# mFinn27/Template-Matching-and-Regression-MapReduce

Measured on AMD Instinct MI355X. Metric: images/sec (whole node) match+regress+NMS; % HBM/MFMA roofline at 1/2/4/8 GPU, higher is better.
Workload: dtype fp32; 1 GPU; config B: 64x SAM feats 256x64x64 (->128x128), 3 exemplars, templates 3x3-15x15, fp32, cls 0.1, IoU 0.5; config=B, images_per_gpu=64, exemplars=3, parallelism=dp1, decoder=split, decoder_precision=fp32

## Files before the change

template-matching-and-regression-mapreduce_amd/csrc/conv_split.hip:

```cpp
#include <algorithm>
#include <type_traits>

#include "tmr_common.h"

namespace {

typedef _Float16 h8 __attribute__((ext_vector_type(8)));
typedef __bf16 b8 __attribute__((ext_vector_type(8)));
typedef float f32x4 __attribute__((ext_vector_type(4)));
typedef __bf16 b4 __attribute__((ext_vector_type(4)));
typedef __attribute__((address_space(3))) void *lds_ptr_t;


constexpr int BM = 128;
constexpr int TH = 16;
constexpr int TW = 32;
constexpr int LDS_KB = 160;
constexpr int PXG = 8, NG = 4;
constexpr int NWAVES = 8;
constexpr int NTHREADS = NWAVES * 64;
constexpr int WNS = (NWAVES == 8 || TH == 8) ? 2 : 1;
static_assert(TH == 4 * NWAVES / WNS, "a wave owns 4 output rows");
constexpr int NIN = 8 / WNS;
constexpr int ACCW = NIN * 8 * 64 * 4;
// ... 473 lines not shown
    if (EPI == 0 && (a.flags & TMR_SPLIT_TILED_OUT)) {
        f32x4 *o = reinterpret_cast<f32x4 *>(
                       a.out + ((((size_t)u * a.NT + nt) * a.MT + mt) * NWAVES + wave) * ACCW) +
                   lane;
#pragma unroll
        for (int in = 0; in < NIN; ++in)
#pragma unroll
            for (int jp = 0; jp < 8; ++jp) {
                __builtin_nontemporal_store(acc[in][jp] * inv, o + (in * 8 + jp) * 64);
            }
        return;
    }
    float *red = reinterpret_cast<float *>(lds);
    float *sb = red + 4 * 8 * NHEAD * 16;
    float *shw = sb + BM;
    if (tid < BM) {
        const int n = nt * BM + tid;
        sb[tid] = n < a.N ? a.bias[n] : 0.0f;
    }
    if (EPI == 1)
        for (int e = tid; e < BM * NHEAD; e += NTHREADS) shw[e] = a.headw[(size_t)nt * BM * NHEAD + e];
    __syncthreads();
    if constexpr (EPI == 0) {
        float invp[8];
#pragma unroll
        for (int jp = 0; jp < 8; ++jp) {
            invp[jp] = inv;
            const int y = ty0 + wpix * 4 + (jp >> 1), x = tx0 + (jp & 1) * 16 + l16;
            if (PR::SCALED && (a.flags & TMR_SPLIT_XMAX_PER_PIXEL) && y < a.H && x < a.W)
                invp[jp] = 1.0f / (split_scale(a.xmax + ((size_t)u * a.H + y) * a.W + x) * split_scale(a.wmax));
        }
#pragma unroll
        for (int in = 0; in < NIN; ++in)
#pragma unroll
            for (int r = 0; r < 4; ++r) {
                const int nl = wn * 64 + in * 16 + 4 * kg + r;
                const int n = nt * BM + nl;
                const bool nin = n < a.N;
                const float bn = sb[nl];
#pragma unroll
                for (int jp = 0; jp < 8; ++jp) {
                    const int y = ty0 + wpix * 4 + (jp >> 1), x = tx0 + (jp & 1) * 16 + l16;
                    float v = acc[in][jp][r] * invp[jp] + bn;
                    if (a.leaky) v = v >= 0.0f ? v : v * 0.01f;
                    if (nin && y < a.H && x < a.W) a.out[((size_t)u * a.N + n) * HW + (size_t)y * a.W + x] = v;
                }
            }
        return;
    }
    f2 hs2[4][NHEAD];
#pragma unroll
    for (int q = 0; q < 4; ++q)
#pragma unroll
        for (int k = 0; k < NHEAD; ++k) hs2[q][k] = (f2){0.0f, 0.0f};
    const f2 inv2 = {inv, inv};
#pragma unroll
    for (int in = 0; in < NIN; ++in)
#pragma unroll
        for (int r = 0; r < 4; ++r) {
            const int nl = wn * 64 + in * 16 + 4 * kg + r;
            const f2 bn2 = {sb[nl], sb[nl]};
            f2 hw2[NHEAD];
#pragma unroll
            for (int k = 0; k < NHEAD; ++k) hw2[k] = (f2){shw[nl * NHEAD + k], shw[nl * NHEAD + k]};
#pragma unroll
            for (int q = 0; q < 4; ++q)
                head_fma(head_act((f2){acc[in][2 * q][r], acc[in][2 * q + 1][r]}, inv2, bn2, a.leaky), hw2, hs2[q]);
            __builtin_amdgcn_sched_barrier(0);
        }
    float X[40];
#pragma unroll
    for (int q = 0; q < 4; ++q)
#pragma unroll
        for (int k = 0; k < NHEAD; ++k) {
            X[2 * (5 * q + k)] = hs2[q][k].x;
            X[2 * (5 * q + k) + 1] = hs2[q][k].y;
        }
    float Y[20], Z[10];
#pragma unroll
    for (int m = 0; m < 20; ++m) {
        const auto s = __builtin_amdgcn_permlane16_swap(__float_as_uint(X[2 * m]), __float_as_uint(X[2 * m + 1]),
                                                         false, false);
        Y[m] = __uint_as_float(s[0]) + __uint_as_float(s[1]);
    }
#pragma unroll
    for (int p = 0; p < 10; ++p) {
        const auto s = __builtin_amdgcn_permlane32_swap(__float_as_uint(Y[2 * p]), __float_as_uint(Y[2 * p + 1]),
                                                         false, false);
        Z[p] = __uint_as_float(s[0]) + __uint_as_float(s[1]);
    }
    __syncthreads();
    if (WNS == 2 && wn == 1) {
#pragma unroll
        for (int p = 0; p < 10; ++p) red[((wpix * 10 + p) * 4 + kg) * 16 + l16] = Z[p];
    }
    __syncthreads();
    if (wn == 0) {
#pragma unroll
        for (int p = 0; p < 10; ++p) {
            const int j = 4 * p + kg, m = j >> 1, q = m / NHEAD, k = m - q * NHEAD;
            const int jp = 2 * q + (j & 1);
            const int y = ty0 + wpix * 4 + (jp >> 1), x = tx0 + (jp & 1) * 16 + l16;
            const float v = Z[p] + (WNS == 2 ? red[((wpix * 10 + p) * 4 + kg) * 16 + l16] : 0.0f);
            if (y < a.H && x < a.W) a.partials[(((size_t)nt * NHEAD + k) * a.U + u) * HW + (size_t)y * a.W + x] = v;
        }
    }
}

template <int KS, int PREC, int EPI>
int launch_split(SArgs a, hipStream_t s) {
    constexpr size_t lds = Geo<KS, PREC>::LDS;
    static_assert(lds <= 160 * 1024, "LDS");
    static_assert((4 * 8 * NHEAD * 16 + BM * (NHEAD + 1)) * 4 <= lds, "epilogue scratch");
    auto kern = split_conv_kernel<KS, PREC, EPI>;
    if (tmr_set_max_lds((const void *)kern, lds) !=
        hipSuccess)
        return TMR_E_HIP;
    const int64_t blocks = (int64_t)a.NTW * a.MT * a.U;
    if (blocks <= 0) return TMR_OK;
    TMR_REQUIRE(blocks < (1ll << 31));
    hipLaunchKernelGGL(kern, dim3((unsigned)blocks), dim3(NTHREADS), lds, s, a);
    TMR_CHECK_LAUNCH();
    return TMR_OK;
}

template <int KS, int EPI>
int dispatch_prec(int prec, const SArgs &a, hipStream_t s) {
    switch (prec) {
        case TMR_PREC_F16X3: return launch_split<KS, TMR_PREC_F16X3, EPI>(a, s);
        case TMR_PREC_BF16: return launch_split<KS, TMR_PREC_BF16, EPI>(a, s);
        case TMR_PREC_F16: return launch_split<KS, TMR_PREC_F16, EPI>(a, s);
        default: return TMR_E_INVALID;
    }
}

template <int EPI>
int dispatch_ks(int ks, int prec, const SArgs &a, hipStream_t s) {
    switch (ks) {
        case 1: return dispatch_prec<1, EPI>(prec, a, s);
        case 3: return dispatch_prec<3, EPI>(prec, a, s);
        case 5: return dispatch_prec<5, EPI>(prec, a, s);
        case 7: return dispatch_prec<7, EPI>(prec, a, s);
        default: return TMR_E_INVALID;
    }
}

constexpr int PT = TMR_POINTS_TILE;
constexpr int PP = 2 * PT;
constexpr int PCG = PP / 16;
constexpr int PTW = NWAVES / WNS;
static_assert(PT == 64 && 4 * PP == NTHREADS, "points block: one store lane per head and point");
static_assert(WNS == 2 && NWAVES == 2 * P, "points block: a wave per 64-channel half; gathers dealt by (piece, half)");

struct PArgs {
    SArgs s;
    const float *head_bias;
    const float *box;
    const int32_t *tiles;
    int ntiles;
    float *b;
};

template <int KS, int PREC>
__global__ __launch_bounds__(NTHREADS) void split_points_kernel(PArgs pa) {
    typedef Prec<PREC> PR;
    typedef typename PR::V V;
    constexpr int T = KS * KS, HALVES = PR::HALVES, WREC = PR::WREC;
    constexpr int NF = NIN;
    constexpr int NS = HALVES == 2 ? 3 * T : T;
    const SArgs &a = pa.s;
    constexpr int BB = T * P * PP * 16;
    extern __shared__ __attribute__((aligned(16))) char plds[];
    char *Bs = plds;
    float(*red)[4][PP] = reinterpret_cast<float(*)[4][PP]>(plds + 2 * BB);
    float(*xch)[4][PP] = reinterpret_cast<float(*)[4][PP]>(plds + BB);
    static_assert(PTW * 4 * PP * sizeof(float) <= BB, "the odd waves' sums fit a B buffer");

    const int tid = threadIdx.x;
    const int lane = tid & 63;
    const int wave = __builtin_amdgcn_readfirstlane(tid >> 6);
    const int wh = wave & 1, wt = wave >> 1;
    const int l16 = lane & 15, kg = lane >> 4;
    const int HW = a.H * a.W;
    int tu[2], tfirst[2], tcnt[2], timg[2];
    float sxw[2];
#pragma unroll
    for (int hh = 0; hh < 2; ++hh) {
        const int64_t ti = 2 * (int64_t)blockIdx.x + hh;
        const bool have = ti < pa.ntiles;
        const int32_t *tl = pa.tiles + 3 * (have ? ti : ti - hh);
        tu[hh] = min(max(tl[0], 0), a.U - 1);
        tfirst[hh] = min(max(tl[1], 0), HW - 1);
        tcnt[hh] = have ? min(max(tl[2], 0), PT) : 0;
        timg[hh] = a.unit_image ? a.unit_image[tu[hh]] : tu[hh];
        sxw[hh] = split_sxw<PREC>(a, tu[hh]);
    }
    const int NC = a.NC0 + a.NC1;
    auto pixel = [&](int u, int first, int cnt, int p) {
        const int *pixi = reinterpret_cast<const int *>(pa.box) + 4 * (size_t)u * HW;
        return min(max(pixi[4 * (size_t)min(first + (p < cnt ? p : 0), HW - 1)], 0), HW - 1);
    };
    const int gu = wh ? tu[1] : tu[0], gfirst = wh ? tfirst[1] : tfirst[0], gcnt = wh ? tcnt[1] : tcnt[0];
    const int gimg = wh ? timg[1] : timg[0];

    const uint32_t cstride = (uint32_t)a.Hp * a.Wp * XREC;
    const int h0 = a.NC0 * HALVES, h1 = a.NC1 * HALVES;
    const __amdgpu_buffer_rsrc_t xr0 = __builtin_amdgcn_make_buffer_rsrc(
        (void *)(h0 ? a.x0 + (size_t)gimg * h0 * cstride : a.x1), (short)0, h0 * cstride, 0x00020000);
    const __amdgpu_buffer_rsrc_t xr1 = __builtin_amdgcn_make_buffer_rsrc(
        (void *)(h1 ? a.x1 + (size_t)gu * h1 * cstride : a.x0), (short)0, h1 * cstride, 0x00020000);
    const uint32_t tapstride = (uint32_t)NC * a.Npad * WREC;
    const __amdgpu_buffer_rsrc_t wr = __builtin_amdgcn_make_buffer_rsrc(
        (void *)a.wp, (short)0, T * tapstride, 0x00020000);
    uint32_t goff[KS];
#pragma unroll
    for (int i = 0; i < KS; ++i) {
        const int g = 64 * i + lane;
        const int pix = pixel(gu, gfirst, gcnt, g / KS), y = pix / a.W;
        goff[i] = (uint32_t)(y * a.Wp + (pix - y * a.W) + g % KS) * 16;
    }
    const uint32_t qstride = (uint32_t)a.Hp * a.Wp * 16;
    auto gather = [&](int hc) {
        const bool s0 = hc < h0;
        const uint32_t hs_ = (uint32_t)(s0 ? hc : hc - h0) * cstride + wt * qstride;
#pragma unroll
        for (int ky = 0; ky < KS; ++ky)
#pragma unroll
            for (int i = 0; i < KS; ++i)
                buffer_lds16(s0 ? xr0 : xr1,
                             (lds_ptr_t)(Bs + (hc & 1) * BB + (((ky * P + wt) * PP + wh * PT) * KS + 64 * i) * 16), goff[i],
                             hs_ + (uint32_t)(ky * a.Wp) * 16);
    };
    const int bfo = kg * (PP * KS * 16) + l16 * (KS * 16);
    auto bfrag = [&](int hc, int tap, int j) -> V {
        return *reinterpret_cast<const V *>(Bs + (hc & 1) * BB + (tap / KS) * (P * PP * KS * 16) + bfo +
                                            j * (16 * KS * 16) + (tap % KS) * 16);
    };

    const int npass = a.NTW > PTW ? 2 : 1;
    for (int pass = 0; pass < npass; ++pass) {
        const int wtile = pass * PTW + wt;
        const bool active = wtile < a.NTW;
        const int nt = a.NT0 + (active ? wtile : 0);
        const uint32_t aoff = (uint32_t)kg * a.Npad * 16 + ((uint32_t)nt * BM + wh * (BM / 2) + l16) * 16;
        gather(0);

        f32x4 acc[NF][PCG];
        if (a.acc_init) {
            const bool i16 = a.flags & TMR_SPLIT_INIT_BF16;
#pragma unroll
            for (int j = 0; j < PCG; ++j) {
                constexpr int HJ = PCG / 2;
                const int hh = j / HJ;
                const int pix = pixel(tu[hh], tfirst[hh], tcnt[hh], (j % HJ) * 16 + l16);
                const int py = pix / a.W, px = pix - py * a.W;
                const float sx = sxw[hh];
                const int islab = (a.flags & TMR_SPLIT_INIT_BCAST) ? 0 : timg[hh];
                const int mt = (py / TH) * a.TXN + px / TW;
                const int wpix = (py % TH) >> 2, jp = ((py & 3) << 1) | ((px % TW) >> 4);
                const size_t g4 = (((((size_t)islab * a.NT + nt) * a.MT + mt) * NWAVES + wpix * WNS + wh) * ACCW) / 4 +
                                  jp * 64 + kg * 16 + (px & 15);
                if (i16) {
                    const b4 *ai = reinterpret_cast<const b4 *>(a.acc_init) + g4;
#pragma unroll
                    for (int f = 0; f < NF; ++f)
                        acc[f][j] = __builtin_convertvector(ai[f * 8 * 64], f32x4) * sx;
                } else {
                    const f32x4 *ai = reinterpret_cast<const f32x4 *>(a.acc_init) + g4;
#pragma unroll
                    for (int f = 0; f < NF; ++f)
                        acc[f][j] = ai[f * 8 * 64] * sx;
                }
            }
        } else {
#pragma unroll
            for (int f = 0; f < NF; ++f)
#pragma unroll
                for (int j = 0; j < PCG; ++j) acc[f][j] = (f32x4){0.0f, 0.0f, 0.0f, 0.0f};
        }

        auto st_part = [](int s) { return HALVES == 2 && s >= 2 * T ? 1 : 0; };
        auto st_tap = [](int s) { return HALVES == 2 ? (s >= 2 * T ? s - 2 * T : s / 2) : s; };
        auto st_term = [](int s) { return HALVES == 2 && s < 2 * T ? s & 1 : 0; };
        auto st_newb = [](int s) { return !(HALVES == 2 && s < 2 * T && (s & 1)); };
        auto st_first = [](int s) { return s == 0 || (HALVES == 2 && s == 2 * T); };
        auto st_last = [](int s) { return s == NS - 1 || (HALVES == 2 && s == 2 * T - 1); };
        constexpr int AR = 3;
        static_assert(NS % AR == 0 && NS >= AR, "weight ring");
        V ar[AR][NF];
        auto load_stage = [&](int c, int s) {
            if (s >= NS) {
                s -= NS;
                c = c + 1 < NC ? c + 1 : c;
            }
            const uint32_t as = (uint32_t)st_tap(s) * tapstride + (uint32_t)c * a.Npad * WREC +
                                (uint32_t)st_term(s) * 4 * a.Npad * 16;
#pragma unroll
            for (int f = 0; f < NF; ++f) ar[s % AR][f] = buffer_load16<V>(wr, aoff + f * 256, as);
        };
#pragma unroll
        for (int s = 0; s < AR - 1; ++s) load_stage(0, s);
        asm volatile("s_waitcnt vmcnt(0)" ::: "memory");
        __syncthreads();
        V bc[PCG];
        const int NHC = NC * HALVES;
        for (int c = 0; c < NC; ++c) {
#pragma unroll
            for (int s = 0; s < NS; ++s) {
                const int hc = c * HALVES + st_part(s);
                load_stage(c, s + AR - 1);
                if (st_first(s)) {
                    if (hc + 1 < NHC) gather(hc + 1);
#pragma unroll
                    for (int j = 0; j < PCG; ++j) bc[j] = bfrag(hc, st_tap(s), j);
                }
                const bool nextb = s + 1 < NS && st_newb(s + 1) && !st_first(s + 1);
                __builtin_amdgcn_sched_barrier(0);
#pragma unroll
                for (int j = 0; j < PCG; ++j) {
#pragma unroll
                    for (int f = 0; f < NF; ++f) acc[f][j] = mma(ar[s % AR][f], bc[j], acc[f][j]);
                    if (nextb) {
                        bc[j] = bfrag(hc, st_tap(s + 1), j);
                        __builtin_amdgcn_sched_barrier(0);
                    }
                }
                __builtin_amdgcn_sched_barrier(0);
                if (st_last(s)) {
                    static_assert((AR - 1) * NF == 8 && T > AR - 1, "the counted wait below");
                    asm volatile("s_waitcnt vmcnt(8)" ::: "memory");
                    __syncthreads();
                }
            }
        }

        f2 hs[PCG / 2][NHEAD];
#pragma unroll
        for (int q = 0; q < PCG / 2; ++q)
#pragma unroll
            for (int k = 0; k < NHEAD; ++k) hs[q][k] = (f2){0.0f, 0.0f};
#pragma unroll
        for (int f = 0; f < NF; ++f)
#pragma unroll
            for (int r = 0; r < 4; ++r) {
                const int n = nt * BM + wh * (BM / 2) + f * 16 + 4 * kg + r;
                const float bv = n < a.N ? a.bias[n] : 0.0f;
                const f2 bn2 = {bv, bv};
                f2 hw2[NHEAD];
#pragma unroll
                for (int k = 0; k < NHEAD; ++k) {
                    const float h = a.headw[(size_t)n * NHEAD + k];
                    hw2[k] = (f2){h, h};
                }
#pragma unroll
                for (int q = 0; q < PCG / 2; ++q) {
                    const float inv = 1.0f / sxw[q / (PCG / 4)];
                    head_fma(head_act((f2){acc[f][2 * q][r], acc[f][2 * q + 1][r]}, (f2){inv, inv}, bn2, a.leaky), hw2,
                             hs[q]);
                }
            }
        float z[PCG / 2][4][2];
#pragma unroll
        for (int q = 0; q < PCG / 2; ++q)
#pragma unroll
            for (int k = 0; k < 4; ++k)
#pragma unroll
                for (int e = 0; e < 2; ++e) {
                    const float x = hs[q][k][e];
                    const float y = x + __shfl_xor(x, 16);
                    z[q][k][e] = y + __shfl_xor(y, 32);
                }
        if (wh == 1 && kg == 0 && active) {
#pragma unroll
            for (int q = 0; q < PCG / 2; ++q)
#pragma unroll
                for (int k = 0; k < 4; ++k)
#pragma unroll
                    for (int e = 0; e < 2; ++e) xch[wt][k][(2 * q + e) * 16 + l16] = z[q][k][e];
        }
        __syncthreads();
        if (wh == 0 && kg == 0 && active) {
#pragma unroll
            for (int q = 0; q < PCG / 2; ++q)
#pragma unroll
                for (int k = 0; k < 4; ++k)
#pragma unroll
                    for (int e = 0; e < 2; ++e) {
                        const int p = (2 * q + e) * 16 + l16;
                        red[wtile][k][p] = z[q][k][e] + xch[wt][k][p];
                    }
        }
    }
    __syncthreads();
    {
        const int k = tid / PP, p = tid % PP, pl = p % PT;
        if (pl < gcnt) {
            const int pix = pixel(gu, gfirst, gcnt, pl);
            float s = 0.0f;
            for (int t = 0; t < a.NTW; ++t) s += red[t][k][p];
            pa.b[((size_t)gu * 4 + k) * HW + pix] = s + pa.head_bias[k];
        }
    }
}

template <int PREC>
int launch_points(const PArgs &pa, int ntiles, hipStream_t s) {
    constexpr size_t lds = 2 * 9 * P * PP * 16 + NWAVES * 4 * PP * sizeof(float);
    static_assert(lds <= LDS_KB * 1024, "LDS");
    auto kern = split_points_kernel<3, PREC>;
    if (tmr_set_max_lds((const void *)kern, lds) != hipSuccess) return TMR_E_HIP;
    hipLaunchKernelGGL(kern, dim3((unsigned)((ntiles + 1) / 2)), dim3(NTHREADS), lds, s, pa);
    TMR_CHECK_LAUNCH();
    return TMR_OK;
}

inline int prec_halves(int prec) { return prec == TMR_PREC_F16X3 ? 2 : 1; }
inline int prec_wrec(int prec) { return prec == TMR_PREC_F16X3 ? 128 : 64; }
inline bool prec_ok(int prec) {
    return prec == TMR_PREC_F16X3 || prec == TMR_PREC_BF16 || prec == TMR_PREC_F16;
}
inline bool ks_ok(int ks) { return ks == 1 || ks == 3 || ks == 5 || ks == 7; }
inline bool tile_window(int flags, int NT, int &first, int &count) {
    first = (flags >> TMR_SPLIT_TILE_FIRST_SHIFT) & 0xff;
    count = (flags >> TMR_SPLIT_TILE_COUNT_SHIFT) & 0x7f;
    if (count == 0) {
        if (first != 0) return false;
        count = NT;
    }
    return first + count <= NT;
}
inline int pad_h(int H, int ks) { return (int)tmr_cdiv(H, TH) * TH + ks - 1; }
inline int pad_w(int W, int ks) { return (int)tmr_cdiv(W, TW) * TW + ks - 1; }

__device__ __forceinline__ void absmax_commit(float m, unsigned *out) {
    __shared__ float red[4];
    for (int o = 32; o > 0; o >>= 1) m = fmaxf(m, __shfl_xor(m, o));
    if ((threadIdx.x & 63) == 0) red[threadIdx.x >> 6] = m;
    __syncthreads();
    if (threadIdx.x == 0) atomicMax(out, __float_as_uint(fmaxf(fmaxf(red[0], red[1]), fmaxf(red[2], red[3]))));
}

__global__ __launch_bounds__(256) void absmax_rows_kernel(const float *__restrict__ x, int64_t n, int vec,
                                                          unsigned *__restrict__ out) {
    const float *xr = x + (size_t)blockIdx.y * n;
    float m = 0.0f;
    const int64_t step = (int64_t)gridDim.x * blockDim.x;
    if (vec) {
        const float4 *x4 = reinterpret_cast<const float4 *>(xr);
        for (int64_t i = (int64_t)blockIdx.x * blockDim.x + threadIdx.x; i < n / 4; i += step) {
            const float4 v = x4[i];
            m = fmaxf(m, fmaxf(fmaxf(fabsf(v.x), fabsf(v.y)), fmaxf(fabsf(v.z), fabsf(v.w))));
        }
    } else {
        for (int64_t i = (int64_t)blockIdx.x * blockDim.x + threadIdx.x; i < n; i += step)
            m = fmaxf(m, fabsf(xr[i]));
    }
    absmax_commit(m, out + blockIdx.y);
}

constexpr int PA_PIX = 64, PA_GRP = 8;
__global__ __launch_bounds__(PA_PIX * PA_GRP) void pixel_absmax_kernel(const float *__restrict__ x, int S, int C,
                                                                       int64_t HW, float *__restrict__ out) {
    __shared__ float part[PA_GRP][PA_PIX];
    const int lane = threadIdx.x & (PA_PIX - 1), grp = threadIdx.x / PA_PIX;
    const int64_t i = (int64_t)blockIdx.x * PA_PIX + lane;
    float m = 0.0f;
    if (i < (int64_t)S * HW) {
        const int64_t s = i / HW, p = i - s * HW;
        const float *xp = x + (size_t)s * C * HW + p;
#pragma unroll 8
        for (int c = grp; c < C; c += PA_GRP) m = fmaxf(m, fabsf(xp[(size_t)c * HW]));
    }
    part[grp][lane] = m;
    __syncthreads();
    if (grp == 0 && i < (int64_t)S * HW) {
#pragma unroll
        for (int g = 1; g < PA_GRP; ++g) m = fmaxf(m, part[g][lane]);
        out[i] = m;
    }
}

__global__ __launch_bounds__(256) void scale_merge_kernel(const float *__restrict__ img_max,
                                                          const float *__restrict__ unit_max,
                                                          const int32_t *__restrict__ unit_image, int U,
                                                          float *__restrict__ out_img,
                                                          float *__restrict__ out_unit) {
    __shared__ float red[4];
    const int b = blockIdx.x;
    float m = 0.0f;
    for (int u = threadIdx.x; u < U; u += blockDim.x)
        if (unit_image[u] == b) m = fmaxf(m, unit_max[u]);
    for (int o = 32; o > 0; o >>= 1) m = fmaxf(m, __shfl_xor(m, o));
    if ((threadIdx.x & 63) == 0) red[threadIdx.x >> 6] = m;
    __syncthreads();
    m = fmaxf(fmaxf(red[0], red[1]), fmaxf(red[2], red[3]));
    if (img_max) m = fmaxf(m, img_max[b]);
    if (threadIdx.x == 0 && out_img) out_img[b] = m;
    for (int u = threadIdx.x; u < U; u += blockDim.x)
        if (unit_image[u] == b) out_unit[u] = m;
}

template <int PREC, int MODE>
__global__ void xpack_kernel(const float *__restrict__ x, int S, int Cin, int Hin, int Win, int ups,
                             int ones, int H, int W, int NCc, int Hp, int Wp, int pad,
                             const float *__restrict__ xmax, int xms,
                             typename Prec<PREC>::V *__restrict__ out) {
    constexpr int HALVES = Prec<PREC>::HALVES;
    const int64_t total = (int64_t)S * NCc * Hp * Wp;
    const int64_t i = (int64_t)blockIdx.x * blockDim.x + threadIdx.x;
    if (i >= total) return;
    const int xp = (int)(i % Wp);
    int64_t r = i / Wp;
    const int yp = (int)(r % Hp);
    r /= Hp;
    const int c = (int)(r % NCc);
    const int s = (int)(r / NCc);
    const int y = yp - pad, xx = xp - pad;
    const bool in = y >= 0 && y < H && xx >= 0 && xx < W;
    const float *xm = !xmax ? nullptr
                      : xms == 2 ? (in ? xmax + ((size_t)s * H + y) * W + xx : nullptr)
                                 : xmax + (size_t)s * xms;
    const float sc = Prec<PREC>::SCALED ? split_scale(xm) : 1.0f;
    float v[CCH];
#pragma unroll
    for (int k = 0; k < CCH; ++k) {
        const int ch = c * CCH + k;
        float val = 0.0f;
        if (in) {
            if (MODE == 0) {
                if (ch < Cin) val = x[(((size_t)s * Cin + ch) * H + y) * W + xx];
            } else if (ch < Cin) {
                const float *pl = x + ((size_t)s * Cin + ch) * Hin * Win;
                val = ups ? up_value(pl, Hin, Win, y, xx) : pl[(size_t)y * Win + xx];
            } else if (ones && ch == Cin) {
                val = 1.0f;
            }
        }
        v[k] = val;
    }
    typename Prec<PREC>::V hi[P], lo[P];
    split_record<PREC>(v, sc, hi, lo);
    const size_t plane = (size_t)Hp * Wp;
    typename Prec<PREC>::V *o = out + ((size_t)s * NCc + c) * HALVES * P * plane + (size_t)yp * Wp + xp;
#pragma unroll
    for (int q = 0; q < P; ++q) o[q * plane] = hi[q];
    if (HALVES == 2) {
#pragma unroll
        for (int q = 0; q < P; ++q) o[(P + q) * plane] = lo[q];
// ... 415 lines not shown
```

template-matching-and-regression-mapreduce_amd/engine.py:

```python
from __future__ import annotations

import contextlib
import weakref
from dataclasses import dataclass
from typing import Dict, Optional, Sequence, Tuple

import numpy as np
import torch

from . import exp_table, graphs, host
from ._lib import (PEAKS_DECODE_ONLY, PEAKS_FIND_ONLY, PEAKS_PROB_SCRATCH, POINTS_TILE, PREC_CODES, SPLIT_OUT_BF16,
                   SPLIT_TILED_OUT, SPLIT_XMAX_PER_PIXEL, UNIT_DTYPE, XCORR_ALGOS, TMRError, call, ptr, require_gpu,
                   size, stream, xcorr)
from .decoder_plan import SCALES_FTM, SCALES_MERGED, HeadsLaunch, decoder_plan
from .graphs import _clone_outputs, _GraphBook, _h2d, _units_to_device
from .operands import absmax
from .operands import (absmax_rows, conv2d_split, fold_proj, pack_split_up, pack_split_w, pack_split_x, pixel_absmax,
                       prec_code, scale_merge)
from .xcorr_cost import mfma_fits, xcorr_choice

NHEAD = 5
NMS_SMALL = 256


# ... 196 lines not shown
        pcode = prec_code(pprec)
        pw, pb = self.P["input_proj.0.weight"], self.P["input_proj.0.bias"]
        N, Cw = pw.shape[0], pw.shape[1]
        if Cw != Cin:
            raise TMRError(f"input_proj expects {Cw} channels, got {Cin}")
        wp, wmax = self._cache.get(f"proj_split_{pprec}", [pw], lambda: pack_split_w(pw, Cin, pprec))
        xmax = None if pprec == "bf16" else pixel_absmax(feats)
        if xmax is not None and self.cfg.precision != "bf16":
            self._memo_absmax(feats, "feat", lambda: absmax_rows(xmax))
        xp = pack_split_up(feats, False, 1, pprec, xmax, ones=False)
        fq = torch.empty((B, N, Hin, Win), device=feats.device, dtype=torch.float32)
        call("tmr_split_conv", ptr(xp), Cin, None, None, 0, B, Hin, Win, 1, pcode, ptr(wp),
             ptr(wmax), ptr(xmax), ptr(pb.detach().float().contiguous()), N, 0, None, None, ptr(fq),
             SPLIT_XMAX_PER_PIXEL if xmax is not None else 0, stream())
        if up:
            fp = torch.empty((B, N, H, W), device=feats.device, dtype=torch.float32)
            call("tmr_upsample2x", ptr(fq), B * N, Hin, Win, ptr(fp), stream())
        else:
            fp = fq
        return fp, (self._f0(feats) if want_f0 else None)

    def _f0(self, feats: torch.Tensor) -> torch.Tensor:
        if not self.cfg.feature_upsample:
            return feats
        B, Cin, Hin, Win = feats.shape
        f0 = torch.empty((B, Cin, 2 * Hin, 2 * Win), device=feats.device, dtype=torch.float32)
        call("tmr_upsample2x", ptr(feats.float().contiguous()), B * Cin, Hin, Win, ptr(f0), stream())
        return f0

    def match(self, fp: torch.Tensor, unit_image: Sequence[int], unit_boxes: np.ndarray,
              want_relu: bool = False, allow_bf16: bool = False):
        B, C, H, W = fp.shape
        U = len(unit_image)
        cfg = self.cfg
        units, tfl, mh, mw = host.build_units(unit_boxes, unit_image, H, W, C, cfg.template_type)
        dev = fp.device
        units_d = _units_to_device(units, dev, tag="units")
        img_units = host.image_ranges(unit_image, B)
        img_units_d = _h2d(np.asarray(img_units), dev, tag="img_units")
        tmpl = torch.empty(max(tfl, 1), device=dev, dtype=torch.float32)
        call("tmr_templates", ptr(fp), B, C, H, W, ptr(units_d), U, mh, mw, ptr(tmpl), stream())
        Co = 1 if cfg.squeeze else C
        work = torch.empty((U, C, H, W), device=dev, dtype=torch.float32) if cfg.squeeze else None
        scale = self.P["matcher.scale"].detach().float().contiguous()
        slots = torch.zeros(U, device=dev, dtype=torch.float32)
        min_k = int(min(units["ht"].min(), units["wt"].min()))
        pc = prec_code(cfg.precision)
        choice = self.xcorr_algo
        if choice == "auto":
            choice = xcorr_choice(units["ht"], units["wt"], U / max(1, len(set(unit_image))),
                                  mfma_fits(W, mh, mw), one_term=pc != PREC_CODES["fp32"])
        self.last_xcorr_algo = choice
        algo = XCORR_ALGOS[choice]
        out16 = (allow_bf16 and self.out_bf16 and pc == PREC_CODES["bf16"] and algo == XCORR_ALGOS["mfma"]
                 and not cfg.squeeze and not want_relu and W % 8 == 0)
        self.last_xcorr_out16 = out16
        out = torch.empty((U, Co, H, W), device=dev, dtype=torch.bfloat16 if out16 else torch.float32)
        relu = torch.empty_like(out) if want_relu else None
        tsplit, rows = None, 0
        if algo != XCORR_ALGOS["valu"] and tfl > 0:
            rows = host.tsplit_rows(units)
            tsplit = torch.empty(size("template_split", U, C, rows), device=dev, dtype=torch.uint8)
            with _timed(self.xcorr_split_events if self.xcorr_events is not None else None):
                call("tmr_template_split", ptr(tmpl), ptr(units_d), U, C, rows, pc, ptr(tsplit), stream())
        with _timed(self.xcorr_events):
            xcorr(f=ptr(fp), templates=ptr(tmpl), units=ptr(units_d), img_units=ptr(img_units_d), scale=ptr(scale),
                  out=ptr(out), relu_out=ptr(relu), work=ptr(work), out_absmax=ptr(slots), tmpl_split=ptr(tsplit),
                  total_rows=rows, B=B, C=C, H=H, W=W, U=U, max_ht=mh, max_wt=mw, squeeze=int(cfg.squeeze),
                  algo=algo, min_k=min_k, prec=pc, out_bf16=int(out16), stream=stream())
        ht, wt = units["ht"].astype(np.float64), units["wt"].astype(np.float64)
        self.last_xcorr_flops = float(np.sum(2.0 * C * (H - ht + 1) * (W - wt + 1) * ht * wt))
        self.last_xcorr_bytes = 2.0 * 4 * C * H * W * U
        nimg = len(set(int(i) for i in unit_image))
        self.last_xcorr_dram_bytes = float(C * H * W) * (4.0 * nimg + (2.0 if out16 else 4.0) * U)
        self._memo_absmax(out, "ftm", lambda: slots)
        return out, relu

    def decode(self, fp: torch.Tensor, f_tm: torch.Tensor, unit_image: Sequence[int],
               feats: Optional[torch.Tensor] = None, box_later: bool = False):
        cfg = self.cfg
        ui = _h2d(np.asarray(unit_image, np.int32), f_tm.device, tag="unit_image")
        if cfg.decoder_num_layer != 1:
            return self._decode_stack(fp, f_tm, ui)
        U, C1, H, W = f_tm.shape
        B, dev = fp.shape[0], f_tm.device
        ks, prec, pc = cfg.decoder_kernel_size, cfg.precision, prec_code(cfg.precision)
        p = decoder_plan(cfg, self.fold_proj, self.share_fp_half, self.reuse_image_work, feats is not None, U, B,
                         unit_image, box_later, self._box_tiles() if box_later else 0)
        Cfp = fp.shape[1] if cfg.fusion else 0
        wp, bias, N, Cw, hw, hb, split, wbias = self._fused_decoders(Cfp if p.share else 0, p.fold)
        if Cw != Cfp + C1:
            raise TMRError(f"decoders expect {Cw} input channels, got {Cfp + C1}")
        C0 = feats.shape[1] if p.fold else Cfp
        bplane = self._bias_plane(wbias, H, W) if p.fold else None
        xmax1 = None if p.unscaled else self._memo_absmax(f_tm, "ftm", lambda: absmax_rows(f_tm))
        xp0 = xmax0 = acc0 = None
        if p.scales != SCALES_FTM:
            xmax0 = None if p.unscaled else self._feat_absmax(feats) if p.fold else absmax_rows(fp)
            if p.scales == SCALES_MERGED and not p.unscaled:
                xmax0, xmax1 = scale_merge(xmax0, xmax1, ui, B)
            if p.share and p.fold:
                acc0 = self._acc0_lookup(feats, split, H, W)
            if acc0 is None:
                xp0 = pack_split_up(feats, cfg.feature_upsample, ks, prec, xmax0, ones=False) if p.fold else \
                    pack_split_x(fp, ks, prec, xmax0)
        xp1 = pack_split_x(f_tm, ks, prec, xmax1)
        if p.share:
            wp_fp, wp, zero_b = split
            if acc0 is None:
                acc0 = torch.empty(size("acc", B, N, H, W), device=dev, dtype=torch.float32)
                call("tmr_split_conv", ptr(xp0), C0, None, None, 0, B, H, W, ks, pc, ptr(wp_fp[0]), ptr(wp_fp[1]),
                     ptr(xmax0), ptr(zero_b), N, 0, None, ptr(bplane), ptr(acc0), p.fp_flags, stream())
                if p.fold and self.reuse_image_work:
                    self._acc0_store(feats, split, H, W, acc0)
        part = torch.empty(size("heads_partials", N, U, H, W), device=dev, dtype=torch.float32)
        heads = HeadsLaunch(xp0=None if p.share else xp0, C0=0 if p.share else C0, ui=ui, xp1=xp1, C1=C1, U=U, H=H, W=W,
                            ks=ks, pc=pc, wp=wp, xmax1=xmax1, bias=bias, N=N, hw=hw, hb=hb,
                            a0=acc0 if p.share else bplane, part=part, plan=p)
        first, count = p.window((N + 127) // 128)
        with _timed(self.decoder_events):
            heads.run(first, count)
        n_run = 128 * count if box_later else N
        self.last_decoder_flops = 2.0 * H * W * n_run * (heads.C0 + C1) * ks ** 2 * U
        self.last_shared_flops = 2.0 * H * W * N * C0 * ks ** 2 * B if p.share else 0.0
        self.last_decoder_algo = "split"
        ob = torch.empty(U * (5 if cfg.box_reg else 1) * H * W, device=dev, dtype=torch.float32)
        o = ob[:U * H * W].view(U, 1, H, W)
        b = ob[U * H * W:].view(U, 4, H, W) if cfg.box_reg else None
        call("tmr_heads_reduce", ptr(part[first * NHEAD * U * H * W:]), n_run, 128, U, H, W, ptr(hb), ptr(o),
             None if box_later else ptr(b), stream())
        if box_later:
            heads.b = b
            self._box_ctx = heads
        return o, b

    def _decode_stack(self, fp, f_tm, ui):
        cfg = self.cfg
        x0 = torch.cat([fp.index_select(0, ui.long()), f_tm], 1) if cfg.fusion else f_tm
        res = {}
        for pre in (["decoder_b"] if cfg.box_reg else []) + ["decoder_o"]:
            x = x0
            for l, (w, bb) in enumerate(self._dec_layers(pre)):
                x = self._conv(f"{pre}.{l}", x, w, bb, True)
            res[pre] = x
        ow, ob = self.P["objectness_head.head.0.weight"], self.P["objectness_head.head.0.bias"]
        o = self._conv("obj", res["decoder_o"], ow, ob, False)
        b = None
        if cfg.box_reg:
            lw, lb = self.P["ltrbs_head.head.0.weight"], self.P["ltrbs_head.head.0.bias"]
            b = self._conv("ltrbs", res["decoder_b"], lw, lb, False)
        return o, b

    box_at_peaks = "auto"
    BOX_POINTS_CROSSOVER = {"fp32": 0.50, "bf16": 0.47, "f16": 0.47}

    def _box_tiles(self) -> int:
        return int(self.P["decoder_b.layer.0.weight"].shape[0]) // 128

    def box_at_peaks_ok(self) -> bool:
        cfg = self.cfg
        if self.box_at_peaks == "never" or cfg.decoder_num_layer != 1 or not cfg.box_reg or \
                cfg.decoder_kernel_size != 3 or self.reuse_image_work:
            return False
        if self.box_at_peaks not in ("auto", "always"):
            raise TMRError("box_at_peaks must be 'auto', 'always' or 'never'")
        nb = int(self.P["decoder_b.layer.0.weight"].shape[0])
        return nb % 128 == 0 and 1 <= nb // 128 <= 8

    def box_at_points(self, box: torch.Tensor, tiles: np.ndarray) -> None:
        if len(tiles):
            td = _h2d(np.ascontiguousarray(tiles, np.int32).reshape(-1), box.device)
            self._box_ctx.run_points(box, td, len(tiles))

    def box_dense(self) -> None:
        h = self._box_ctx
        nbt = h.plan.skip_tiles
        h.run(0, nbt)
        scratch_o = torch.empty(h.U * h.H * h.W, device=h.b.device, dtype=torch.float32)
        call("tmr_heads_reduce", ptr(h.part), 128 * nbt, 128, h.U, h.H, h.W, ptr(h.hb), ptr(scratch_o), ptr(h.b),
             stream())

    def _detect_box_at_peaks(self, feats, unit_image, boxes, params):
        r = self._forward_units_eager(feats, [int(i) for i in unit_image], boxes, box_later=True)
        o, b = r["o"], r["b"]
        U, _, H, W = o.shape
        logits, box, ref, counts, _ = self.peaks(o, None, params, want_prob=False, phase="find")
        counts_host = counts.cpu().numpy()
        need = np.where(params["mode"] != 2, counts_host, 0)
        self.last_points = int(need.sum())
        dense = self.box_at_peaks == "auto" and \
            self.last_points > self.BOX_POINTS_CROSSOVER[self.cfg.precision] * U * H * W
        self.last_box_route = "dense" if dense else "points"
        if dense:
            self.box_dense()
            self.last_points_flops = 0.0
        else:
            tiles = host.point_tiles(need, POINTS_TILE)
            self.box_at_points(box, tiles)
            h = self._box_ctx
            self.last_points_flops = 2.0 * 128 * h.plan.skip_tiles * (h.C0 + h.C1) * h.ks ** 2 * POINTS_TILE * len(tiles)
        self._box_ctx = None
        self.peaks(o, b, params, want_prob=False, phase="decode", found=(logits, box, ref, counts))
        return logits, box, ref, counts, counts_host

    def _proj_key(self):
        params = (self.P["input_proj.0.weight"], self.P["input_proj.0.bias"])
        return params, (_version_key(params), self.cfg.precision, self.cfg.feature_upsample)

    def _bind_memo(self, feats: torch.Tensor, fp, split=None, size_=None, acc0=None):
        params, pkey = self._proj_key()
        self._memo = _ImageMemo(weakref.ref(feats), feats._version, feats.data_ptr(), pkey,
                                tuple(weakref.ref(t) for t in params), fp, split, size_, acc0)

    def _fp_lookup(self, feats: torch.Tensor):
        m = self._memo
        params, pkey = self._proj_key()
        hit = m is not None and m.is_for(feats) and m.fp is not None and m.pkey == pkey and \
            all(r() is t for r, t in zip(m.params, params))
        return m.fp if hit else None

    def _acc0_lookup(self, feats, split, H, W):
        m = self._memo
        hit = self.reuse_image_work and m is not None and m.is_for(feats) and m.split is split and m.size == (H, W)
        return m.acc0 if hit else None

    def _acc0_store(self, feats, split, H, W, acc0):
        m = self._memo
        if m is not None and m.is_for(feats):
            m.split, m.size, m.acc0 = split, (H, W), acc0
        else:
            self._bind_memo(feats, None, split, (H, W), acc0)

    def _memo_hit(self, feats: torch.Tensor) -> Optional[_ImageMemo]:
        return self._memo if self._fp_lookup(feats) is not None and self._memo.acc0 is not None else None

    def _forward_units_graphed(self, feats, unit_image, unit_boxes, want_aux):
        if not (self.use_graphs and feats.is_cuda and len(unit_image) <= self.GRAPH_MAX_UNITS) or \
                self.decoder_events is not None or self.xcorr_events is not None or self.cfg.no_matcher or \
                self.cfg.decoder_num_layer != 1 or not (self.cfg.fusion and self.fold_proj):
            return None
        B, Cin, Hin, Win = feats.shape
        H, W = (2 * Hin, 2 * Win) if self.cfg.feature_upsample else (Hin, Win)
        C = int(self.P["input_proj.0.weight"].shape[0])
        boxes = np.asarray(unit_boxes, np.float32).reshape(-1, 4)
        units = host.build_units(boxes, unit_image, H, W, C, self.cfg.template_type)[0]
        hit = self._memo_hit(feats)
        base = self._graph_signature(feats, units, unit_image, False, False, module=True)
        if base is None:
            return None
        sig = base + (bool(want_aux), None if hit is None else (hit.fp.data_ptr(), hit.acc0.data_ptr()))
        g = self._graphs.get(sig)
        self.last_graph = "replay" if g is not None else "eager"
        if g is None:
            if not self._graphs.want_capture(sig):
                return None
            g = self._capture_module(feats, unit_image, boxes, want_aux, hit, self._detect_host_inputs(
                units, unit_image, B, np.zeros(0, np.uint8)))
            self._graphs.put(sig, g)
            if g is None:
                return None
            self.last_graph = "captured"
        host_in = self._detect_host_inputs(units, unit_image, B, np.zeros(0, np.uint8))
        out = g.replay(self, feats.float().contiguous(), host_in, reuse_feats=True)
        if hit is None:
            m = g.memo
            self._bind_memo(feats, m.fp, m.split, m.size, m.acc0)
        return _clone_outputs(out)

    def _capture_module(self, feats, unit_image, boxes, want_aux, hit, host_in):
        saved = self._memo

        def run(static):
            if hit is not None:
                self._bind_memo(static, hit.fp, hit.split, hit.size, hit.acc0)
            else:
                self._memo = None
            return self._forward_units_eager(static, unit_image, boxes, want_aux)

        try:
            g = graphs.capture(self, feats, host_in, run)
            if g is not None and hit is None:
                g.memo = self._memo
                if g.memo is None or g.memo.acc0 is None:
                    self.last_graph_error, g = "the image's first call kept no fp half: the signature stays eager", None
        finally:
            self._memo = saved
        return g

    def forward_units(self, feats: torch.Tensor, unit_image: Sequence[int], unit_boxes,
                      want_aux: bool = False):
        unit_image = [int(i) for i in unit_image]
        if self.reuse_image_work and not graphs.capturing():
            r = self._forward_units_graphed(feats, unit_image, unit_boxes, want_aux)
            if r is not None:
                return r
        return self._forward_units_eager(feats, unit_image, unit_boxes, want_aux)

    def _forward_units_eager(self, feats: torch.Tensor, unit_image: Sequence[int], unit_boxes,
                             want_aux: bool = False, box_later: bool = False):
        fp = self._fp_lookup(feats) if self.reuse_image_work else None
        if fp is not None:
            f0 = self._f0(feats) if want_aux else None
        else:
            fp, f0 = self.project(feats, want_f0=want_aux)
            if self.reuse_image_work:
                m = self._memo
                self._bind_memo(feats, fp, *((m.split, m.size, m.acc0) if m is not None and m.is_for(feats) else ()))
# ... 256 lines not shown
```

Baseline: 705.0 images/s.

## Cut register pressure and spills in split points kernel K-loop

New measurement: 712.8 images/s, median of 6. 1.1% higher.

```diff
diff --git a/profiles/kernel_resources.py b/profiles/kernel_resources.py
--- /dev/null
+++ b/profiles/kernel_resources.py
@@ -0,0 +1,74 @@
+import json
+import os
+import re
+import subprocess
+import sys
+import tempfile
+
+REPO = os.path.dirname(os.path.dirname(os.path.abspath(__file__)))
+sys.path.insert(0, REPO)
+from tmr_import import load_package
+
+CSRC = os.path.join(REPO, "template-matching-and-regression-mapreduce_amd", "csrc")
+OUT = os.path.join(REPO, "profiles", "points_kloop", "resources.json")
+PRECS = {0: "F16X3", 1: "BF16", 2: "F16"}
+PARENT = {
+    "F16X3": {"vgprs": 256, "vgpr_spills": 146, "scratch_bytes_per_lane": 252, "occupancy": 2},
+    "BF16": {"vgprs": 256, "vgpr_spills": 10, "scratch_bytes_per_lane": 44, "occupancy": 2},
+    "F16": {"vgprs": 256, "vgpr_spills": 110, "scratch_bytes_per_lane": 204, "occupancy": 2},
+}
+FIELDS = {"VGPRs": "vgprs", "AGPRs": "agprs", "VGPRs Spill": "vgpr_spills", "SGPRs Spill": "sgpr_spills",
+          "ScratchSize [bytes/lane]": "scratch_bytes_per_lane", "Occupancy [waves/SIMD]": "occupancy"}
+
+
+def makefile_flags():
+    var = {"EXTRA": ""}
+    for line in open(os.path.join(CSRC, "Makefile")):
+        m = re.match(r"^(\w+)\s*\??=\s*(.*)$", line.rstrip("\n"))
+        if m and m.group(1) not in var:
+            var[m.group(1)] = m.group(2)
+    expand = lambda s: re.sub(r"\$\((\w+)\)", lambda m: expand(var.get(m.group(1), "")), s)
+    return os.environ.get("HIPCC", expand(var["HIPCC"])), expand(var["FLAGS"]).split()
+
+
+def remarks(hipcc, flags):
+    with tempfile.TemporaryDirectory() as tmp:
+        cmd = [hipcc, *flags, "--cuda-device-only", "-Rpass-analysis=kernel-resource-usage", "-c",
+               os.path.join(CSRC, "conv_split.hip"), "-o", os.path.join(tmp, "conv_split.o")]
+        return subprocess.run(cmd, check=True, capture_output=True, text=True).stderr
+
+
+def parse(text):
+    out, cur = {}, None
+    for line in text.splitlines():
+        m = re.search(r"remark: +([^:]+): (.*?) \[-Rpass-analysis", line)
+        if not m:
+            continue
+        key, val = m.group(1).strip(), m.group(2).strip()
+        if key == "Function Name":
+            k = re.search(r"split_points_kernelILi3ELi(\d)EE", val)
+            cur = out.setdefault(PRECS[int(k.group(1))], {}) if k else None
+        elif cur is not None and key in FIELDS:
+            cur[FIELDS[key]] = int(val)
+    return out
+
+
+def main():
+    out_path = sys.argv[1] if len(sys.argv) > 1 else OUT
+    hipcc, flags = makefile_flags()
+    kernels = parse(remarks(hipcc, flags))
+    assert sorted(kernels) == sorted(PRECS.values()), kernels
+    load_package()
+    from tmr_amd import buildinfo
+    rec = {"kernel": "split_points_kernel<3, PREC>", "flags": flags, "source_digest": buildinfo.source_digest("heads"),
+           "kernels": kernels, "parent": PARENT}
+    os.makedirs(os.path.dirname(out_path), exist_ok=True)
+    with open(out_path, "w") as f:
+        json.dump(rec, f, indent=1)
+        f.write("\n")
+    for p, k in kernels.items():
+        print(p, json.dumps(k))
+
+
+if __name__ == "__main__":
+    main()
diff --git a/template-matching-and-regression-mapreduce_amd/csrc/conv_split.hip b/template-matching-and-regression-mapreduce_amd/csrc/conv_split.hip
--- a/template-matching-and-regression-mapreduce_amd/csrc/conv_split.hip
+++ b/template-matching-and-regression-mapreduce_amd/csrc/conv_split.hip
@@ -649,6 +649,16 @@
 static_assert(PT == 64 && 4 * PP == NTHREADS, "points block: one store lane per head and point");
 static_assert(WNS == 2 && NWAVES == 2 * P, "points block: a wave per 64-channel half; gathers dealt by (piece, half)");
 
+__device__ __forceinline__ int lane_now() {
+    int l;
+    asm volatile("v_mbcnt_lo_u32_b32 %0, -1, 0\n\tv_mbcnt_hi_u32_b32 %0, -1, %0" : "=v"(l));
+    return l;
+}
+__device__ __forceinline__ int lane_read(int v, int src) { return __builtin_amdgcn_ds_bpermute(src << 2, v); }
+__device__ __forceinline__ float lane_read(float v, int src) {
+    return __builtin_bit_cast(float, lane_read(__builtin_bit_cast(int, v), src));
+}
+
 struct PArgs {
     SArgs s;
     const float *head_bias;
@@ -686,13 +696,14 @@
         const int64_t ti = 2 * (int64_t)blockIdx.x + hh;
         const bool have = ti < pa.ntiles;
         const int32_t *tl = pa.tiles + 3 * (have ? ti : ti - hh);
-        tu[hh] = min(max(tl[0], 0), a.U - 1);
-        tfirst[hh] = min(max(tl[1], 0), HW - 1);
-        tcnt[hh] = have ? min(max(tl[2], 0), PT) : 0;
-        timg[hh] = a.unit_image ? a.unit_image[tu[hh]] : tu[hh];
-        sxw[hh] = split_sxw<PREC>(a, tu[hh]);
-    }
-    const int NC = a.NC0 + a.NC1;
+        tu[hh] = __builtin_amdgcn_readfirstlane(min(max(tl[0], 0), a.U - 1));
+        tfirst[hh] = __builtin_amdgcn_readfirstlane(min(max(tl[1], 0), HW - 1));
+        tcnt[hh] = __builtin_amdgcn_readfirstlane(have ? min(max(tl[2], 0), PT) : 0);
+        timg[hh] = __builtin_amdgcn_readfirstlane(a.unit_image ? a.unit_image[tu[hh]] : tu[hh]);
+        sxw[hh] = __builtin_bit_cast(
+            float, __builtin_amdgcn_readfirstlane(__builtin_bit_cast(int, split_sxw<PREC>(a, tu[hh]))));
+    }
+    const int NC = a.NC0 + a.NC1, NHC = NC * HALVES;
     auto pixel = [&](int u, int first, int cnt, int p) {
         const int *pixi = reinterpret_cast<const int *>(pa.box) + 4 * (size_t)u * HW;
         return min(max(pixi[4 * (size_t)min(first + (p < cnt ? p : 0), HW - 1)], 0), HW - 1);
@@ -702,31 +713,37 @@
 
     const uint32_t cstride = (uint32_t)a.Hp * a.Wp * XREC;
     const int h0 = a.NC0 * HALVES, h1 = a.NC1 * HALVES;
-    const __amdgpu_buffer_rsrc_t xr0 = __builtin_amdgcn_make_buffer_rsrc(
-        (void *)(h0 ? a.x0 + (size_t)gimg * h0 * cstride : a.x1), (short)0, h0 * cstride, 0x00020000);
-    const __amdgpu_buffer_rsrc_t xr1 = __builtin_amdgcn_make_buffer_rsrc(
-        (void *)(h1 ? a.x1 + (size_t)gu * h1 * cstride : a.x0), (short)0, h1 * cstride, 0x00020000);
+    auto uniform_ptr = [](const char *p) {
+        const uint64_t v = (uint64_t)p;
+        return (const char *)((uint64_t)(uint32_t)__builtin_amdgcn_readfirstlane((int)(uint32_t)v) |
+                              (uint64_t)(uint32_t)__builtin_amdgcn_readfirstlane((int)(uint32_t)(v >> 32)) << 32);
+    };
+    const char *xb0 = uniform_ptr(h0 ? a.x0 + (size_t)gimg * h0 * cstride : a.x1);
+    const char *xb1 = uniform_ptr(h1 ? a.x1 + (size_t)gu * h1 * cstride : a.x0);
     const uint32_t tapstride = (uint32_t)NC * a.Npad * WREC;
     const __amdgpu_buffer_rsrc_t wr = __builtin_amdgcn_make_buffer_rsrc(
         (void *)a.wp, (short)0, T * tapstride, 0x00020000);
+    const int gpix0 = pixel(gu, gfirst, gcnt, lane);
     uint32_t goff[KS];
 #pragma unroll
     for (int i = 0; i < KS; ++i) {
         const int g = 64 * i + lane;
-        const int pix = pixel(gu, gfirst, gcnt, g / KS), y = pix / a.W;
+        const int pix = lane_read(gpix0, g / KS), y = pix / a.W;
         goff[i] = (uint32_t)(y * a.Wp + (pix - y * a.W) + g % KS) * 16;
     }
     const uint32_t qstride = (uint32_t)a.Hp * a.Wp * 16;
-    auto gather = [&](int hc) {
-        const bool s0 = hc < h0;
-        const uint32_t hs_ = (uint32_t)(s0 ? hc : hc - h0) * cstride + wt * qstride;
+    auto gather = [&](int hc, bool live = true) {
+        const int hcl = min(hc, NHC - 1);
+        const bool s0 = hcl < h0;
+        const uint32_t hs_ = (uint32_t)(s0 ? hcl : hcl - h0) * cstride + wt * qstride;
+        const __amdgpu_buffer_rsrc_t xr = __builtin_amdgcn_make_buffer_rsrc(
+            (void *)(s0 ? xb0 : xb1), (short)0, live ? (s0 ? h0 : h1) * cstride : 0, 0x00020000);
 #pragma unroll
         for (int ky = 0; ky < KS; ++ky)
 #pragma unroll
             for (int i = 0; i < KS; ++i)
-                buffer_lds16(s0 ? xr0 : xr1,
-                             (lds_ptr_t)(Bs + (hc & 1) * BB + (((ky * P + wt) * PP + wh * PT) * KS + 64 * i) * 16), goff[i],
-                             hs_ + (uint32_t)(ky * a.Wp) * 16);
+                buffer_lds16(xr, (lds_ptr_t)(Bs + (hc & 1) * BB + (((ky * P + wt) * PP + wh * PT) * KS + 64 * i) * 16),
+                             goff[i], hs_ + (uint32_t)(ky * a.Wp) * 16);
     };
     const int bfo = kg * (PP * KS * 16) + l16 * (KS * 16);
     auto bfrag = [&](int hc, int tap, int j) -> V {
@@ -739,41 +756,67 @@
         const int wtile = pass * PTW + wt;
         const bool active = wtile < a.NTW;
         const int nt = a.NT0 + (active ? wtile : 0);
-        const uint32_t aoff = (uint32_t)kg * a.Npad * 16 + ((uint32_t)nt * BM + wh * (BM / 2) + l16) * 16;
+        const int lp = lane_now(), l16p = lp & 15, kgp = lp >> 4;
+        uint32_t aoff = (uint32_t)kgp * a.Npad * 16 + ((uint32_t)nt * BM + wh * (BM / 2) + l16p) * 16;
         gather(0);
 
         f32x4 acc[NF][PCG];
         if (a.acc_init) {
-            const bool i16 = a.flags & TMR_SPLIT_INIT_BF16;
-#pragma unroll
-            for (int j = 0; j < PCG; ++j) {
-                constexpr int HJ = PCG / 2;
+            constexpr int HJ = PCG / 2;
+            int Wd = a.W, fl = a.flags;
+            asm volatile("" : "+s"(Wd), "+s"(fl));
+            const int ppix[2] = {pixel(tu[0], tfirst[0], tcnt[0], lp), pixel(tu[1], tfirst[1], tcnt[1], lp)};
+            auto group4 = [&](int j) {
                 const int hh = j / HJ;
-                const int pix = pixel(tu[hh], tfirst[hh], tcnt[hh], (j % HJ) * 16 + l16);
-                const int py = pix / a.W, px = pix - py * a.W;
-                const float sx = sxw[hh];
-                const int islab = (a.flags & TMR_SPLIT_INIT_BCAST) ? 0 : timg[hh];
+                const int pix = lane_read(ppix[hh], (j % HJ) * 16 + l16p);
+                const int py = pix / Wd, px = pix - py * Wd;
+                const int islab = (fl & TMR_SPLIT_INIT_BCAST) ? 0 : timg[hh];
                 const int mt = (py / TH) * a.TXN + px / TW;
                 const int wpix = (py % TH) >> 2, jp = ((py & 3) << 1) | ((px % TW) >> 4);
-                const size_t g4 = (((((size_t)islab * a.NT + nt) * a.MT + mt) * NWAVES + wpix * WNS + wh) * ACCW) / 4 +
-                                  jp * 64 + kg * 16 + (px & 15);
-                if (i16) {
-                    const b4 *ai = reinterpret_cast<const b4 *>(a.acc_init) + g4;
+                static_assert(ACCW / 4 == 1 << 11 && 8 * 64 <= ACCW / 4, "the shifts below");
+                const uint32_t row = (uint32_t)(mt * NWAVES + wpix * WNS + wh), in = jp * 64 + kgp * 16 + (px & 15);
+                typedef uint32_t u2 __attribute__((ext_vector_type(2)));
+                u2 lh = {row << 11 | in, row >> 21};
+                asm volatile("" : "+v"(lh));
+                return ((size_t)islab * a.NT + nt) * a.MT * NWAVES * (ACCW / 4) + __builtin_bit_cast(uint64_t, lh);
+            };
+            if (fl & TMR_SPLIT_INIT_BF16) {
+#pragma unroll
+                for (int j = 0; j < PCG; ++j) {
+                    const b4 *ai = reinterpret_cast<const b4 *>(a.acc_init) + group4(j);
+#pragma unroll
+                    for (int f = 0; f < NF; ++f) {
+                        const f2 raw = __builtin_bit_cast(f2, ai[f * 8 * 64]);
+                        acc[f][j] = (f32x4){raw.x, raw.y, 0.0f, 0.0f};
+                    }
+                    __builtin_amdgcn_sched_barrier(0);
+                }
+#pragma unroll
+                for (int j = 0; j < PCG; ++j)
 #pragma unroll
                     for (int f = 0; f < NF; ++f)
-                        acc[f][j] = __builtin_convertvector(ai[f * 8 * 64], f32x4) * sx;
-                } else {
-                    const f32x4 *ai = reinterpret_cast<const f32x4 *>(a.acc_init) + g4;
-#pragma unroll
-                    for (int f = 0; f < NF; ++f)
-                        acc[f][j] = ai[f * 8 * 64] * sx;
+                        acc[f][j] = __builtin_convertvector(__builtin_bit_cast(b4, (f2){acc[f][j][0], acc[f][j][1]}),
+                                                            f32x4) * sxw[j / HJ];
+            } else {
+#pragma unroll
+                for (int j = 0; j < PCG; ++j) {
+                    const f32x4 *ai = reinterpret_cast<const f32x4 *>(a.acc_init) + group4(j);
+#pragma unroll
+                    for (int f = 0; f < NF; ++f) acc[f][j] = ai[f * 8 * 64];
+                    __builtin_amdgcn_sched_barrier(0);
                 }
+#pragma unroll
+                for (int j = 0; j < PCG; ++j)
+#pragma unroll
+                    for (int f = 0; f < NF; ++f) acc[f][j] = acc[f][j] * sxw[j / HJ];
             }
         } else {
+            float zf = 0.0f;
+            asm volatile("" : "+v"(zf));
 #pragma unroll
             for (int f = 0; f < NF; ++f)
 #pragma unroll
-                for (int j = 0; j < PCG; ++j) acc[f][j] = (f32x4){0.0f, 0.0f, 0.0f, 0.0f};
+                for (int j = 0; j < PCG; ++j) acc[f][j] = (f32x4){zf, zf, zf, zf};
         }
 
         auto st_part = [](int s) { return HALVES == 2 && s >= 2 * T ? 1 : 0; };
@@ -785,13 +828,14 @@
         constexpr int AR = 3;
         static_assert(NS % AR == 0 && NS >= AR, "weight ring");
         V ar[AR][NF];
+        uint32_t ts = tapstride, npl = (uint32_t)a.Npad * 16;
         auto load_stage = [&](int c, int s) {
             if (s >= NS) {
                 s -= NS;
                 c = c + 1 < NC ? c + 1 : c;
             }
-            const uint32_t as = (uint32_t)st_tap(s) * tapstride + (uint32_t)c * a.Npad * WREC +
-                                (uint32_t)st_term(s) * 4 * a.Npad * 16;
+            const uint32_t as = (uint32_t)st_tap(s) * ts + (uint32_t)c * npl * (WREC / 16) +
+                                (uint32_t)st_term(s) * 4 * npl;
 #pragma unroll
             for (int f = 0; f < NF; ++f) ar[s % AR][f] = buffer_load16<V>(wr, aoff + f * 256, as);
         };
@@ -799,26 +843,31 @@
         for (int s = 0; s < AR - 1; ++s) load_stage(0, s);
         asm volatile("s_waitcnt vmcnt(0)" ::: "memory");
         __syncthreads();
-        V bc[PCG];
-        const int NHC = NC * HALVES;
+        constexpr int BW = HALVES == 2 ? PCG : PCG / 2;
+        static_assert(PCG % BW == 0, "a group's slot is j % BW in every stage");
+        V bc[BW];
         for (int c = 0; c < NC; ++c) {
+            asm volatile("" : "+v"(aoff));
+            asm volatile("" : "+s"(ts), "+s"(npl));
 #pragma unroll
             for (int s = 0; s < NS; ++s) {
                 const int hc = c * HALVES + st_part(s);
                 load_stage(c, s + AR - 1);
                 if (st_first(s)) {
-                    if (hc + 1 < NHC) gather(hc + 1);
-#pragma unroll
-                    for (int j = 0; j < PCG; ++j) bc[j] = bfrag(hc, st_tap(s), j);
+                    gather(hc + 1, hc + 1 < NHC);
+#pragma unroll
+                    for (int j = 0; j < BW; ++j) bc[j] = bfrag(hc, st_tap(s), j);
                 }
-                const bool nextb = s + 1 < NS && st_newb(s + 1) && !st_first(s + 1);
                 __builtin_amdgcn_sched_barrier(0);
 #pragma unroll
                 for (int j = 0; j < PCG; ++j) {
 #pragma unroll
-                    for (int f = 0; f < NF; ++f) acc[f][j] = mma(ar[s % AR][f], bc[j], acc[f][j]);
-                    if (nextb) {
-                        bc[j] = bfrag(hc, st_tap(s + 1), j);
+                    for (int f = 0; f < NF; ++f) acc[f][j] = mma(ar[s % AR][f], bc[j % BW], acc[f][j]);
+                    if (j + BW < PCG) {
+                        bc[j % BW] = bfrag(hc, st_tap(s), j + BW);
+                        __builtin_amdgcn_sched_barrier(0);
+                    } else if (!st_last(s) && (BW < PCG || st_newb(s + 1))) {
+                        bc[j % BW] = bfrag(hc, st_tap(s + 1), j + BW - PCG);
                         __builtin_amdgcn_sched_barrier(0);
                     }
                 }
@@ -831,31 +880,49 @@
             }
         }
 
+        const int le = lane_now(), kge = le >> 4, l16e = le & 15;
+        float se[2] = {sxw[0], sxw[1]};
+        asm volatile("" : "+s"(se[0]), "+s"(se[1]));
         f2 hs[PCG / 2][NHEAD];
 #pragma unroll
         for (int q = 0; q < PCG / 2; ++q)
 #pragma unroll
             for (int k = 0; k < NHEAD; ++k) hs[q][k] = (f2){0.0f, 0.0f};
-#pragma unroll
-        for (int f = 0; f < NF; ++f)
+        float bvs[2][4], hws[2][4][NHEAD];
+        auto load_hw = [&](int f) {
 #pragma unroll
             for (int r = 0; r < 4; ++r) {
-                const int n = nt * BM + wh * (BM / 2) + f * 16 + 4 * kg + r;
-                const float bv = n < a.N ? a.bias[n] : 0.0f;
+                const int n = nt * BM + wh * (BM / 2) + f * 16 + 4 * kge + r;
+                const float bl = a.bias[min(n, a.N - 1)];
+                bvs[f & 1][r] = n < a.N ? bl : 0.0f;
+#pragma unroll
+                for (int k = 0; k < NHEAD; ++k) hws[f & 1][r][k] = a.headw[(size_t)n * NHEAD + k];
+            }
+        };
+        load_hw(0);
+#pragma unroll
+        for (int f = 0; f < NF; ++f) {
+            if (f + 1 < NF) load_hw(f + 1);
+            __builtin_amdgcn_sched_barrier(0);
+#pragma unroll
+            for (int r = 0; r < 4; ++r) {
+                const float bv = bvs[f & 1][r];
                 const f2 bn2 = {bv, bv};
                 f2 hw2[NHEAD];
 #pragma unroll
                 for (int k = 0; k < NHEAD; ++k) {
-                    const float h = a.headw[(size_t)n * NHEAD + k];
+                    const float h = hws[f & 1][r][k];
                     hw2[k] = (f2){h, h};
                 }
 #pragma unroll
                 for (int q = 0; q < PCG / 2; ++q) {
-                    const float inv = 1.0f / sxw[q / (PCG / 4)];
+                    const float inv = 1.0f / se[q / (PCG / 4)];
                     head_fma(head_act((f2){acc[f][2 * q][r], acc[f][2 * q + 1][r]}, (f2){inv, inv}, bn2, a.leaky), hw2,
                              hs[q]);
                 }
             }
+            __builtin_amdgcn_sched_barrier(0);
+        }
         float z[PCG / 2][4][2];
 #pragma unroll
         for (int q = 0; q < PCG / 2; ++q)
@@ -864,33 +931,34 @@
 #pragma unroll
                 for (int e = 0; e < 2; ++e) {
                     const float x = hs[q][k][e];
-                    const float y = x + __shfl_xor(x, 16);
-                    z[q][k][e] = y + __shfl_xor(y, 32);
+                    const float y = x + lane_read(x, le ^ 16);
+                    z[q][k][e] = y + lane_read(y, le ^ 32);
                 }
-        if (wh == 1 && kg == 0 && active) {
+        if (wh == 1 && kge == 0 && active) {
 #pragma unroll
             for (int q = 0; q < PCG / 2; ++q)
 #pragma unroll
                 for (int k = 0; k < 4; ++k)
 #pragma unroll
-                    for (int e = 0; e < 2; ++e) xch[wt][k][(2 * q + e) * 16 + l16] = z[q][k][e];
+                    for (int e = 0; e < 2; ++e) xch[wt][k][(2 * q + e) * 16 + l16e] = z[q][k][e];
         }
         __syncthreads();
-        if (wh == 0 && kg == 0 && active) {
+        if (wh == 0 && kge == 0 && active) {
 #pragma unroll
             for (int q = 0; q < PCG / 2; ++q)
 #pragma unroll
                 for (int k = 0; k < 4; ++k)
 #pragma unroll
                     for (int e = 0; e < 2; ++e) {
-                        const int p = (2 * q + e) * 16 + l16;
+                        const int p = (2 * q + e) * 16 + l16e;
                         red[wtile][k][p] = z[q][k][e] + xch[wt][k][p];
                     }
         }
     }
     __syncthreads();
     {
-        const int k = tid / PP, p = tid % PP, pl = p % PT;
+        const int te = wave * 64 + lane_now();
+        const int k = te / PP, p = te % PP, pl = p % PT;
         if (pl < gcnt) {
             const int pix = pixel(gu, gfirst, gcnt, pl);
             float s = 0.0f;
diff --git a/template-matching-and-regression-mapreduce_amd/engine.py b/template-matching-and-regression-mapreduce_amd/engine.py
--- a/template-matching-and-regression-mapreduce_amd/engine.py
+++ b/template-matching-and-regression-mapreduce_amd/engine.py
@@ -372,7 +372,7 @@
         return o, b
 
     box_at_peaks = "auto"
-    BOX_POINTS_CROSSOVER = {"fp32": 0.50, "bf16": 0.47, "f16": 0.47}
+    BOX_POINTS_CROSSOVER = {"fp32": 0.57, "bf16": 0.47, "f16": 0.47}
 
     def _box_tiles(self) -> int:
         return int(self.P["decoder_b.layer.0.weight"].shape[0]) // 128
```
